# falcon-computing/falcon-genome

Measured on AMD Instinct MI355X. Metric: PairHMM GCUPS + banded-SW GCUPS per GPU; end-to-end htc regions/sec at 8 GPUs, higher is better.
Workload: dtype fp32 (fp64 rescue)

## Files before the change

falcon-genome_amd/csrc/fcship_api.cpp:

```cpp
#include <hip/hip_runtime.h>
#include <rocprim/device/device_radix_sort.hpp>

#include <algorithm>
#include <chrono>
#include <cmath>
#include <cstdlib>
#include <cstring>
#include <map>
#include <memory>
#include <condition_variable>
#include <mutex>
#include <thread>
#include <vector>

#include "fcship_internal.h"

namespace fcs {

static thread_local std::string g_last_error;
static thread_local int64_t g_last_rescued = 0;
static thread_local double g_last_device_ms = 0, g_last_rescue_ms = 0;
void set_error(const std::string& msg) { g_last_error = msg; }
int fail(int code, const std::string& msg) {
  set_error(msg);
// ... 469 lines not shown
  d.dq = b->read_dq;
  d.gq = b->read_gcp;
  d.read_off = b->read_off;
  d.read_len = b->read_len;
  d.hb = b->hap_bases;
  d.hap_off = b->hap_off;
  d.hap_len = b->hap_len;
  d.pair_read = b->pair_read;
  d.pair_hap = b->pair_hap;
  d.n_pairs = b->n_pairs;
  return d;
}

static int check_batch_shape(const fcs_phmm_batch* b) {
  if (!b) return fail(FCS_ERR_INVALID, "[E::fcship] null PairHMM batch");
  if (b->n_pairs < 0 || b->n_reads < 0 || b->n_haps < 0)
    return fail(FCS_ERR_INVALID, "[E::fcship] negative PairHMM batch size");
  if (b->n_pairs > 0x7FFFFFFF) return fail(FCS_ERR_UNSUPPORTED, "[E::fcship] more than 2^31-1 pairs per batch");
  if (b->n_pairs > 0 && (!b->read_bases || !b->read_bq || !b->read_iq || !b->read_dq || !b->read_gcp ||
                         !b->read_off || !b->read_len || !b->hap_bases || !b->hap_off || !b->hap_len ||
                         !b->pair_read || !b->pair_hap))
    return fail(FCS_ERR_INVALID, "[E::fcship] null pointer in PairHMM batch");
  if (b->max_hap_len < 0 || b->max_read_len < 0)
    return fail(FCS_ERR_INVALID, "[E::fcship] negative max length in PairHMM batch");
  return FCS_OK;
}

extern "C" {

const char* fcs_last_error(void) { return g_last_error.c_str(); }
const char* fcs_version(void) { return "fcship 0.1.0 (gfx950)"; }

int fcs_device_count(void) {
  int n = 0;
  if (hipGetDeviceCount(&n) != hipSuccess) return 0;
  return n;
}

int fcs_set_default_device(int32_t device) {
  int rc = check_device(device);
  if (rc) return rc;
  g_default_device = device;
  return FCS_OK;
}

void fcs_phmm_opts_default(fcs_phmm_opts* o) {
  if (!o) return;
  o->device = 0;
  o->use_fp64_rescue = 1;
  o->rescue_threshold = 1e-28f;
  o->exact_order = 0;
}

void fcs_bsw_params_default(fcs_bsw_params* p) {
  if (!p) return;
  for (int i = 0, k = 0; i < 4; ++i) {
    for (int j = 0; j < 4; ++j) p->mat[k++] = (int8_t)(i == j ? 1 : -4);
    p->mat[k++] = -1;
  }
  for (int j = 0; j < 5; ++j) p->mat[20 + j] = -1;
  p->o_del = 6;
  p->e_del = 1;
  p->o_ins = 6;
  p->e_ins = 1;
  p->end_bonus = 5;
  p->zdrop = 100;
}

int fcs_phmm_plan_create(int32_t device, int64_t max_pairs, fcs_phmm_plan** plan) {
  if (!plan || max_pairs < 0) return fail(FCS_ERR_INVALID, "[E::fcs_phmm_plan_create] bad arguments");
  int rc = check_device(device);
  if (rc) return rc;
  FCS_SET_DEVICE((device));
  DeviceTables* t = nullptr;
  rc = get_device_tables(device, &t);
  if (rc) return rc;
  std::unique_ptr<fcs_phmm_plan> p(new fcs_phmm_plan());
  p->device = device;
  p->max_pairs = max_pairs;
  const size_t n = (size_t)std::max<int64_t>(max_pairs, 1);
  FCS_HIP_CHECK(hipMalloc(&p->idx_out, n * 4));
  FCS_HIP_CHECK(hipMalloc(&p->rescue_list, n * 4));
  FCS_HIP_CHECK(hipMalloc(&p->fb_list, n * 4));
  FCS_HIP_CHECK(hipMalloc(&p->rescue_count, (2 + kPhmmLaunchClasses + 1) * sizeof(unsigned long long)));
  p->fb_count = p->rescue_count + 1;
  p->bounds = reinterpret_cast<int64_t*>(p->rescue_count + 2);
  constexpr size_t kBins = (size_t)1 << (kPhmmKeyBits - 4);
  FCS_HIP_CHECK(hipMalloc(&p->bin_hist, 2 * kBins * sizeof(uint32_t)));
  p->bin_cursor = p->bin_hist + kBins;
  *plan = p.release();
  return FCS_OK;
}

int fcs_phmm_plan_destroy(fcs_phmm_plan* p) {
  if (!p) return FCS_OK;
  ::fcs::DeviceScope dev_scope;
  (void)hipSetDevice(p->device);
  (void)hipFree(p->idx_out);
  (void)hipFree(p->rescue_list);
  (void)hipFree(p->fb_list);
  (void)hipFree(p->rescue_count);
  (void)hipFree(p->bin_hist);
  delete p;
  return FCS_OK;
}

int fcs_phmm_dev_schedule(fcs_phmm_plan* plan, const fcs_phmm_batch* b, void* stream) {
  if (!plan) return fail(FCS_ERR_INVALID, "[E::fcs_phmm_dev_schedule] null plan");
  int rc = check_batch_shape(b);
  if (rc) return rc;
  if (b->n_pairs > plan->max_pairs) return fail(FCS_ERR_INVALID, "[E::fcs_phmm_dev_schedule] batch exceeds plan");
  FCS_SET_DEVICE((plan->device));
  hipStream_t s = (hipStream_t)stream;
  const PhmmDevBatch d = to_dev(b);
  plan->scheduled = -1;
  if (!plan->bin_zeroed)
    FCS_HIP_CHECK(hipMemsetAsync(plan->bin_hist, 0, ((size_t)1 << (kPhmmKeyBits - 4)) * sizeof(uint32_t), s));
  plan->bin_zeroed = false;
  if ((rc = launch_phmm_bin_schedule(d, plan->idx_out, plan->bounds, plan->rescue_count, plan->bin_hist,
                                     plan->bin_cursor, s)))
    return rc;
  plan->bin_zeroed = true;
  plan->counters_zeroed = true;
  if (fault_drop_schedule()) FCS_HIP_CHECK(hipMemsetAsync(plan->bounds, 0, (kPhmmLaunchClasses + 1) * sizeof(int64_t), s));
  plan->scheduled = b->n_pairs;
  return FCS_OK;
}

int fcs_phmm_dev_forward(fcs_phmm_plan* plan, const fcs_phmm_batch* b, double* out, const fcs_phmm_opts* opts,
                         void* stream) {
  if (!plan || !opts) return fail(FCS_ERR_INVALID, "[E::fcs_phmm_dev_forward] null plan/opts");
  int rc = check_batch_shape(b);
  if (rc) return rc;
  if (plan->scheduled != b->n_pairs)
    return fail(FCS_ERR_INVALID, "[E::fcs_phmm_dev_forward] batch not scheduled (call fcs_phmm_dev_schedule)");
  if (b->n_pairs > 0 && !out) return fail(FCS_ERR_INVALID, "[E::fcs_phmm_dev_forward] null output");
  FCS_SET_DEVICE((plan->device));
  DeviceTables* t = nullptr;
  rc = get_device_tables(plan->device, &t);
  if (rc) return rc;
  hipStream_t s = (hipStream_t)stream;
  if (!plan->counters_zeroed)
    FCS_HIP_CHECK(hipMemsetAsync(plan->rescue_count, 0, 2 * sizeof(unsigned long long), s));
  plan->counters_zeroed = false;
  return launch_phmm_forward(to_dev(b), plan->idx_out, b->n_pairs, std::max(b->max_hap_len, 1), plan->bounds, *t,
                             opts->exact_order != 0, out, plan->rescue_list, plan->rescue_count,
                             opts->rescue_threshold, opts->use_fp64_rescue != 0, plan->fb_list, plan->fb_count, s);
}

int fcs_phmm_dev_rescue(fcs_phmm_plan* plan, const fcs_phmm_batch* b, double* out, const fcs_phmm_opts* opts,
                        void* stream) {
  if (!plan || !opts) return fail(FCS_ERR_INVALID, "[E::fcs_phmm_dev_rescue] null plan/opts");
  int rc = check_batch_shape(b);
  if (rc) return rc;
  if (!opts->use_fp64_rescue) return FCS_OK;
  FCS_SET_DEVICE((plan->device));
  DeviceTables* t = nullptr;
  rc = get_device_tables(plan->device, &t);
  if (rc) return rc;
  return launch_phmm_rescue(to_dev(b), plan->rescue_list, plan->rescue_count, b->n_pairs,
                            std::max(b->max_hap_len, 1), *t, opts->exact_order != 0, out, (hipStream_t)stream);
}

int fcs_phmm_dev_run(fcs_phmm_plan* plan, const fcs_phmm_batch* b, double* out, const fcs_phmm_opts* opts,
                     void* stream) {
  int rc = fcs_phmm_dev_schedule(plan, b, stream);
  if (rc) return rc;
  rc = fcs_phmm_dev_forward(plan, b, out, opts, stream);
  if (rc) return rc;
  return fcs_phmm_dev_rescue(plan, b, out, opts, stream);
}

int fcs_stream_release(int32_t device, void* stream) {
  int rc = check_device(device);
  if (rc) return rc;
  FCS_SET_DEVICE((device));
  ForkSet f;
  BswWorkspace ws;
  bool have_fork = false;
  {
    std::lock_guard<std::mutex> lk(g_fork_mu);
    auto wi = g_stream_ws->find({device, (hipStream_t)stream});
    if (wi != g_stream_ws->end()) {
      ws = wi->second;
      g_stream_ws->erase(wi);
    }
    auto it = g_fork_sets->find({device, (hipStream_t)stream});
    if (it != g_fork_sets->end()) {
      f = it->second;
      g_fork_sets->erase(it);
      have_fork = true;
    }
  }
  if (ws.keys_in) {
    (void)hipStreamSynchronize((hipStream_t)stream);
    ws_free(ws);
  }
  if (!have_fork) return FCS_OK;
  hipError_t first = hipSuccess;
  const char* what = nullptr;
  auto note = [&](hipError_t e, const char* w) {
    if (e != hipSuccess && first == hipSuccess) first = e, what = w;
  };
  for (int i = 0; i < kForkStreams - 1; ++i) {
    note(hipStreamSynchronize(f.side[i]), "hipStreamSynchronize");
    note(hipStreamDestroy(f.side[i]), "hipStreamDestroy");
    note(hipEventDestroy(f.join[i]), "hipEventDestroy");
  }
  note(hipEventDestroy(f.fork), "hipEventDestroy");
  if (first != hipSuccess)
    return fail(FCS_ERR_DEVICE, std::string("[E::fcs_stream_release] ") + what + ": " + hipGetErrorString(first));
  return FCS_OK;
}

int fcs_device_warmup(int32_t device, int32_t sessions) {
  int rc = check_device(device);
  if (rc) return rc;
  static const uint8_t b[1] = {'A'}, q[1] = {30}, g[1] = {10}, iq[1] = {45};
  const fcs_phmm_read r{b, q, iq, iq, g, 1};
  const fcs_phmm_hap h{b, 1};
  double out = 0;
  fcs_phmm_opts o;
  fcs_phmm_opts_default(&o);
  o.device = device;
  if ((rc = fcs_phmm_compute(&r, 1, &h, 1, &out, &o))) return rc;
  FCS_SET_DEVICE((device));
  return prefill_sessions(device, sessions <= 0 ? sessions_per_device() : sessions);
}

int fcs_phmm_last_device_ms(double* device_ms, double* rescue_ms) {
// ... 1066 lines not shown
```

falcon-genome_amd/csrc/fcship_internal.h:

```cpp
#pragma once

#include <hip/hip_runtime.h>
#include <stdint.h>

#include <string>

#include "fcship.h"

namespace fcs {

void set_error(const std::string& msg);
int fail(int code, const std::string& msg);
#define FCS_HIP_CHECK(expr)                                                                  \
  do {                                                                                       \
    hipError_t _e = (expr);                                                                  \
    if (_e != hipSuccess)                                                                    \
      return ::fcs::fail(FCS_ERR_DEVICE, std::string("[E::fcship] ") + #expr + ": " +        \
                                             hipGetErrorString(_e));                         \
  } while (0)

struct DeviceScope {
  int prev = -1;
  DeviceScope() {
    if (hipGetDevice(&prev) != hipSuccess) prev = -1;
// ... 33 lines not shown
  const long long o = __double_as_longlong(old), s = __double_as_longlong(src);
  const int lo = __builtin_amdgcn_update_dpp((int)o, (int)s, kDppRowShr1, 0xF, 0xF, false);
  const int hi = __builtin_amdgcn_update_dpp((int)(o >> 32), (int)(s >> 32), kDppRowShr1, 0xF, 0xF, false);
  return __longlong_as_double(((long long)hi << 32) | (unsigned int)lo);
}
template <typename T> __device__ __forceinline__ T dpp_row_shr1(T old, T src);
template <> __device__ __forceinline__ float dpp_row_shr1<float>(float old, float src) { return dpp_row_shr1_f(old, src); }
template <> __device__ __forceinline__ double dpp_row_shr1<double>(double old, double src) { return dpp_row_shr1_d(old, src); }

__device__ __forceinline__ int dpp_wave_shr1_i(int old, int src) {
  return __builtin_amdgcn_update_dpp(old, src, kDppWaveShr1, 0xF, 0xF, false);
}

__device__ __forceinline__ int wave_incl_max(int v, int neg) {
  v = max(v, __builtin_amdgcn_update_dpp(neg, v, kDppRowShr1, 0xF, 0xF, false));
  v = max(v, __builtin_amdgcn_update_dpp(neg, v, kDppRowShr2, 0xF, 0xF, false));
  v = max(v, __builtin_amdgcn_update_dpp(neg, v, kDppRowShr4, 0xF, 0xF, false));
  v = max(v, __builtin_amdgcn_update_dpp(neg, v, kDppRowShr8, 0xF, 0xF, false));
  v = max(v, __builtin_amdgcn_update_dpp(neg, v, kDppRowBcast15, 0xA, 0xF, false));
  v = max(v, __builtin_amdgcn_update_dpp(neg, v, kDppRowBcast31, 0xC, 0xF, false));
  return v;
}

__device__ __forceinline__ int lane_id() { return (int)__lane_id(); }

__device__ __forceinline__ int read_lane(int v, int lane) { return __builtin_amdgcn_readlane(v, lane); }
__device__ __forceinline__ int first_lane(int v) { return __builtin_amdgcn_readfirstlane(v); }

__device__ __forceinline__ int wave_max(int v) {
  return read_lane(wave_incl_max(v, INT32_MIN), 63);
}

__host__ __device__ __forceinline__ int bwa_max_gap(int qlen, int max_mat, int end_bonus, int o, int e) {
  if (e <= 0) return 0x7FFFFFFF;
  const int n = qlen * max_mat + end_bonus - o;
  const int m = (n + e) / e;
  return m > 1 ? m : 1;
}

template <typename T>
struct PhmmTables {
  const T* ph2pr;
  const T* dmatch;
  const T* dmis;
  const T* mm;
  T init_const;
  T log10_init;
};
constexpr int kMmEntries = (127 * 128) / 2 + 128;

struct PhmmDevBatch {
  const uint8_t *rb, *bq, *iq, *dq, *gq;
  const int64_t* read_off;
  const int32_t* read_len;
  const uint8_t* hb;
  const int64_t* hap_off;
  const int32_t* hap_len;
  const int32_t* pair_read;
  const int32_t* pair_hap;
  int64_t n_pairs;
};

struct DeviceTables {
  bool ready = false;
  float* f_tabs = nullptr;
  double* d_tabs = nullptr;
  PhmmTables<float> tf;
  PhmmTables<double> td;
};
int get_device_tables(int device, DeviceTables** out);

void build_phmm_tables_f(float* ph2pr, float* dmatch, float* dmis, float* mm);
void build_phmm_tables_d(double* ph2pr, double* dmatch, double* dmis, double* mm);

constexpr int kForkStreams = 4;
int fork_streams(hipStream_t s, hipStream_t (&fs)[kForkStreams]);
int join_streams(hipStream_t s, const hipStream_t (&fs)[kForkStreams]);

int launch_phmm_bin_schedule(const PhmmDevBatch& b, int32_t* idx_out, int64_t* bounds, unsigned long long* counters,
                             uint32_t* hist, uint32_t* cursor, hipStream_t s);
int launch_phmm_forward(const PhmmDevBatch& b, const int32_t* order, int64_t count, int max_hap_len,
                        const int64_t* bounds, const DeviceTables& t, bool exact, double* out, int32_t* rescue_list,
                        unsigned long long* rescue_count, float thr, bool use_rescue, int32_t* fb_list,
                        unsigned long long* fb_count, hipStream_t s);
int launch_phmm_rescue(const PhmmDevBatch& b, const int32_t* list, const unsigned long long* count_dev,
                       int64_t max_count, int max_hap_len, const DeviceTables& t, bool exact, double* out,
                       hipStream_t s);

struct BswDevBatch {
  const uint8_t* qbuf;
  const int64_t* qoff;
  const int32_t* qlen;
  const uint8_t* tbuf;
  const int64_t* toff;
  const int32_t* tlen;
  const int32_t* h0;
  const int32_t* w;
  int64_t n;
};
struct BswParams {
  int8_t mat[25];
  int32_t o_del, e_del, o_ins, e_ins, end_bonus, zdrop;
  int32_t max_mat;
  int32_t matpack[5];
  int32_t lane_ok;
  int32_t pair_ok;
  int32_t pair_bias;
  int32_t pair_cg;
  int32_t pair_k256, pair_one;
};
constexpr int kBswPairBucket0 = 10;
constexpr int kBswWideBucket = 15;
struct BswWorkspace {
  int64_t cap = 0;
  uint32_t* keys_in = nullptr;
  uint32_t* keys_out = nullptr;
  int32_t* idx_in = nullptr;
  int32_t* idx_out = nullptr;
  int64_t* bounds = nullptr;
  void* tmp = nullptr;
  size_t tmp_bytes = 0;
};
hipError_t sort_pairs_u32(void* tmp, size_t& bytes, const uint32_t* kin, uint32_t* kout, const int32_t* vin,
                          int32_t* vout, int n, hipStream_t s, int end_bit = 32);
constexpr int kBswKeyBucketShift = 20;
constexpr int kBswKeyBits = 24;
constexpr int kPhmmKeyClassShift = 12;
constexpr int kPhmmKeyBits = 16;
constexpr int kStreamClasses = 4;
constexpr int kPhmmClasses = 6;
constexpr int kLongClasses = 2;
constexpr int kColsLaunch = 8;
constexpr int kPhmmLaunchClasses = kLongClasses + kColsLaunch + kPhmmClasses;
int launch_bsw_extend_sorted(const BswDevBatch& b, const BswParams& p, int max_qlen, int max_tlen, int32_t* res,
                             int64_t* cells, const BswWorkspace& ws, hipStream_t s);
int launch_bsw_extend_wide(const BswDevBatch& b, const BswParams& p, int max_qlen, int max_tlen, int32_t* res,
                           int64_t* cells, const int32_t* order, const int64_t* bounds, hipStream_t s);
int launch_bsw_align(const BswDevBatch& b, const BswParams& p, const int32_t* xtra, int max_qlen, int max_tlen,
                     int32_t* out, hipStream_t s, bool all_u8);
int launch_bsw_global(const BswDevBatch& b, const BswParams& p, int max_qlen, int max_tlen, int32_t* scores,
                      uint8_t* zbuf, int64_t zbytes, const int64_t* zoff, uint32_t* cigar, const int64_t* cigar_off,
                      const int32_t* cigar_cap, int32_t* n_cigar, hipStream_t s);
int launch_bgzf_inflate(const uint8_t* comp, const int64_t* coff, const int64_t* uoff, int32_t n, uint8_t* out,
                        int32_t* status, hipStream_t s);

}
```

falcon-genome_amd/csrc/phmm_cols.h:

```cpp
#pragma once

namespace fcs {

constexpr int kColsClasses = 8;
constexpr int kColsMinR = 33;
__host__ __device__ constexpr int cols_C(int c) { return c == 0 ? 19 : 18 - c; }
__host__ __device__ constexpr int cols_hmax(int c) { return 16 * cols_C(c) - 1; }
__host__ __device__ inline int cols_class(int H) {
  for (int c = kColsClasses - 1; c >= 0; --c)
    if (H <= cols_hmax(c)) return c;
  return -1;
}
constexpr int kColsRing = 32;
constexpr int kColsChunks = 6;
constexpr int kColsChunkBytes = kColsRing * 4 * 16;
constexpr int kColsCapOff = kColsChunks * kColsChunkBytes;
constexpr int kColsTabOff = kColsCapOff + 4 * 8 * 8;
constexpr int kColsLds = kColsTabOff + 3 * 128 * 4;

__device__ __forceinline__ uint32_t vconst(uint32_t k) {
  uint32_t r;
  asm volatile("v_mov_b32 %0, %1" : "=v"(r) : "i"(k));
  return r;
}
// ... 657 lines not shown
          }
          asm volatile("" ::: "memory");
          const uint32_t a0 = xs + (uint32_t)(S * 8);
          const uint32_t pa = min(a0, a0 - (uint32_t)(kCols1Ring * 8)) + segoff;
          auto ld2 = [&](int chunk) {
            return *reinterpret_cast<const __attribute__((address_space(3))) pf2*>((uintptr_t)(pa + chunk * kCols1ChunkBytes));
          };
          const pf2 r0 = ld2(0), r1 = ld2(1), r2 = ld2(2), r3 = ld2(3);
          const pu2 cr = *reinterpret_cast<const __attribute__((address_space(3))) pu2*>((uintptr_t)(pa + 4 * kCols1ChunkBytes));
          const float e1 = r0.x, e3 = r0.y, my = r1.x, yy = r1.y, mm = r2.x, gm = r2.y, mx = r3.x, xx = r3.y;
          const float z = (float)(cr.y >> 24);
          const float din = __int_as_float(__builtin_amdgcn_update_dpp(__float_as_int(z), __float_as_int(dn), kDppRowShr1, 0xF, 0xF, false));
          const float xnx = __int_as_float(__builtin_amdgcn_update_dpp(__float_as_int(z), __float_as_int(xo), kDppRowShr1, 0xF, 0xF, false));
          const float xcur = xin;
          xin = xnx;
          uint32_t mA = 0;
          auto prior = [&](int j, const float dep) {
            if ((j & 3) == 0) mA = __builtin_amdgcn_perm(cr.y, cr.x, cur[j >> 2]);
            int a;
            asm volatile("v_bfe_i32 %0, %1, %2, 1" : "=v"(a) : "v"(mA), "i"(8 * (j & 3)), "v"(dep));
            return sel_v((uint32_t)a, e1, e3);
          };
          float Mn = xcur * prior(0, xcur);
          float D = din, Mp = 0.f, Dp = 0.f;
#pragma unroll
          for (int j = 0; j < C; ++j) {
            const float M = Mn;
            if (j > 0) D = __builtin_fmaf(Mp, my, Dp * yy);
            float I = In[j], Xo = Xn[j];
            asm volatile("" : "+v"(I), "+v"(Xo) : "v"(D));
            if (j + 1 < C) Mn = Xo * prior(j + 1, D);
            float xn = __builtin_fmaf(M, mm, __builtin_fmaf(I, gm, D));
            float in = __builtin_fmaf(M, mx, I * xx);
            asm volatile("" : "+v"(xn), "+v"(in));
            Xn[j] = xn;
            In[j] = in;
            Mp = M;
            Dp = D;
          }
          dn = __builtin_fmaf(Mp, my, Dp * yy);
          xo = Xn[C - 1];
          uint64_t keep;
          const uint32_t cpa = capa + 0u;
          const float dnv = dn;
          asm volatile(
              "s_mov_b64 %0, exec\n\t"
              "s_mov_b64 exec, %3\n\t"
              "ds_write_b32 %1, %2 offset:%4\n\t"
              "s_mov_b64 exec, %0"
              : "=&s"(keep)
              : "v"(cpa), "v"(dnv), "s"(kTopLanes), "i"(4 * S)
              : "memory");
        };
        [&]<int... S>(std::integer_sequence<int, S...>) {
          (step(std::integral_constant<int, S>{}), ...);
        }(std::make_integer_sequence<int, 8>{});
        g0 += 8;
        swmask >>= 8;
        capa += 32;
        xs += 64;
        xs = min(xs, xs - (uint32_t)(kCols1Ring * 8));
      }
      if (any_cap) {
        if (sl == 15 && (unsigned)(cap - gb) < 16u) {
          const float acc = *reinterpret_cast<const float*>(smem_raw + kCols1CapOff + seg * 64 + 4 * (cap - gb));
          const int p = capp;
          if (capo) {
            const unsigned long long k = atomicAdd(fb_count, 1ull);
            fb_list[k] = p;
            out[p] = __builtin_nan("");
          } else if (use_rescue && acc < thr) {
            const unsigned long long k = atomicAdd(rescue_count, 1ull);
            rescue_list[k] = p;
            out[p] = __builtin_nan("");
          } else {
            out[p] = (double)(log10f(acc) - tab.log10_init);
          }
        }
      }
    }
  }
}

}
```

falcon-genome_amd/csrc/phmm_kernels.hip:

```cpp
#include <hip/hip_runtime.h>

#include <algorithm>
#include <cstdlib>
#include <cstring>

#include <utility>

#include "fcship_internal.h"

namespace fcs {

constexpr int PFD = 2;
template <typename T> struct alignas(2 * sizeof(T)) PhRing {
  T X, I;
};

__device__ __forceinline__ float fma_t(float a, float b, float c) { return fmaf(a, b, c); }
__device__ __forceinline__ double fma_t(double a, double b, double c) { return fma(a, b, c); }

__device__ __forceinline__ unsigned char base_code(unsigned char b) {
  return b == 'A' ? 0 : b == 'C' ? 1 : b == 'G' ? 2 : b == 'T' ? 3 : b == 'N' ? 4 : 5;
}
__device__ __forceinline__ int base_mask(int rb) {
  const int c = base_code((unsigned char)rb);
// ... 287 lines not shown
        if (bytecmp)
          phmm_stripe<T, EXACT, true, true, W>(sp, ring, hapl, sl, (tend + 16) >> 4, lim, ulim, accM, accI, tab, nraw, nprm, top);
        else
          phmm_stripe<T, EXACT, true, false, W>(sp, ring, hapl, sl, (tend + 16) >> 4, lim, ulim, accM, accI, tab, nraw, nprm, top);
        if (seg_sums && sl == sum_lane) {
          const T sum = accM + accI;
          if constexpr (RESCUE_PASS) {
            out[p] = log10(sum) - (double)tab.log10_init;
          } else {
            if (use_rescue && sum < (T)thr) {
              const unsigned long long k = atomicAdd(rescue_count, 1ull);
              rescue_list[k] = p;
              out[p] = __builtin_nan("");
            } else {
              out[p] = (double)(log10f((float)sum) - (float)tab.log10_init);
            }
          }
        }
      } else {
        if (bytecmp)
          phmm_stripe<T, EXACT, false, true, W>(prm, ring, hapl, sl, (Hmax + W + 15) >> 4, -1, -1, accM, accI, tab, nraw, nprm, top);
        else
          phmm_stripe<T, EXACT, false, false, W>(prm, ring, hapl, sl, (Hmax + W + 15) >> 4, -1, -1, accM, accI, tab, nraw, nprm, top);
      }
      prm = nprm;
    }
  }
}

}

#include "phmm2.h"
#include "phmm_stream.h"
#include "phmm_cols.h"

namespace fcs {

static __host__ __device__ int nslot_for(int max_hap_len) { return ((max_hap_len + 51 + 15) / 16) * 16; }
static __host__ __device__ int nslot_for_w(int max_hap_len, int W) {
  return ((max_hap_len + 2 * W + 19 + 15) / 16) * 16;
}

static_assert(kPhmmLaunchClasses <= 16 && kPhmmKeyClassShift + 4 <= kPhmmKeyBits, "class fits the key");
__host__ __device__ inline int phmm_class(int H) {
  const int c = (nslot_for(H) - 224 + 31) / 32;
  return c < 0 ? 0 : c > kPhmmClasses - 1 ? kPhmmClasses - 1 : c;
}

__host__ __device__ inline int phmm_launch_class(int R, int H, int& stream_cls) {
  stream_cls = -1;
  if (R >= kStreamMinR && R <= kStreamMaxR && H >= 1) {
    static_assert(kColsMinR <= kStreamMinR, "column-blocked streams take every streamed read");
    const int cc = cols_class(H);
    stream_cls = cc >= 0 ? 0 : stream_class(H);
    if (cc >= 0) return kLongClasses + cc;
    if (stream_cls >= 2) return kStreamClasses - 1 - stream_cls;
    stream_cls = -1;
  }
  return kLongClasses + kColsLaunch + kPhmmClasses - 1 - phmm_class(max(H, 0));
}

__device__ __forceinline__ uint32_t phmm_key(const PhmmDevBatch& b, long long p) {
  const int R = b.read_len[b.pair_read[p]];
  const int H = b.hap_len[b.pair_hap[p]];
  int sc;
  const uint32_t cf = (uint32_t)phmm_launch_class(R, H, sc);
  const uint32_t hh = 0xFFFu - (uint32_t)min(max(H, 0), 0xFFF);
  uint32_t low;
  if (sc >= 0)
    low = hh;
  else
    low = ((3u - (uint32_t)min((max(R, 0) + 15) >> 4, 3)) << 10) | (0x3FFu - (uint32_t)min(max(H, 0) >> 2, 0x3FF));
  return (cf << kPhmmKeyClassShift) | low;
}

constexpr int kPhmmBins = 1 << (kPhmmKeyBits - 4);
constexpr int kBinBlock = 1024, kBinItems = 4;
__device__ __forceinline__ int phmm_bin(const PhmmDevBatch& b, long long p) { return (int)(phmm_key(b, p) >> 4); }

__global__ __launch_bounds__(kBinBlock) void phmm_bin_count_kernel(const PhmmDevBatch b, uint32_t* __restrict__ hist,
                                                                    unsigned long long* __restrict__ counters) {
  __shared__ uint32_t h[kPhmmBins];
  for (int i = threadIdx.x; i < kPhmmBins; i += kBinBlock) h[i] = 0;
  if (blockIdx.x == 0 && threadIdx.x == 0) {
    counters[0] = 0ull;
    counters[1] = 0ull;
  }
  __syncthreads();
  const long long base = (long long)blockIdx.x * (kBinBlock * kBinItems);
  for (int k = 0; k < kBinItems; ++k) {
    const long long p = base + (long long)k * kBinBlock + threadIdx.x;
    if (p < b.n_pairs) atomicAdd(&h[phmm_bin(b, p)], 1u);
  }
  __syncthreads();
  for (int i = threadIdx.x; i < kPhmmBins; i += kBinBlock)
    if (h[i]) atomicAdd(&hist[i], h[i]);
}

__global__ __launch_bounds__(kBinBlock) void phmm_bin_scan_kernel(uint32_t* __restrict__ hist,
                                                                   uint32_t* __restrict__ cursor, long long n,
                                                                   int64_t* __restrict__ bounds) {
  constexpr int kPer = kPhmmBins / kBinBlock;
  __shared__ uint32_t part[kBinBlock];
  const int t = threadIdx.x;
  uint32_t v[kPer], sum = 0;
  for (int j = 0; j < kPer; ++j) {
    v[j] = hist[t * kPer + j];
    sum += v[j];
  }
  part[t] = sum;
  __syncthreads();
  for (int off = 1; off < kBinBlock; off <<= 1) {
    const uint32_t x = t >= off ? part[t - off] : 0u;
    __syncthreads();
    part[t] += x;
    __syncthreads();
  }
  uint32_t run = part[t] - sum;
  for (int j = 0; j < kPer; ++j) {
    const int bin = t * kPer + j;
    cursor[bin] = run;
    if ((bin & 255) == 0 && (bin >> 8) < kPhmmLaunchClasses) bounds[bin >> 8] = run;
    run += v[j];
    hist[bin] = 0u;
  }
  if (t == 0) bounds[kPhmmLaunchClasses] = n;
}

__global__ __launch_bounds__(kBinBlock) void phmm_bin_scatter_kernel(const PhmmDevBatch b,
                                                                      uint32_t* __restrict__ cursor,
                                                                      int32_t* __restrict__ idx) {
  __shared__ uint32_t cnt[kPhmmBins], at[kPhmmBins];
  for (int i = threadIdx.x; i < kPhmmBins; i += kBinBlock) cnt[i] = 0;
  __syncthreads();
  const long long base = (long long)blockIdx.x * (kBinBlock * kBinItems);
  int bin[kBinItems];
  uint32_t rank[kBinItems];
  for (int k = 0; k < kBinItems; ++k) {
    const long long p = base + (long long)k * kBinBlock + threadIdx.x;
    bin[k] = p < b.n_pairs ? phmm_bin(b, p) : -1;
    rank[k] = bin[k] >= 0 ? atomicAdd(&cnt[bin[k]], 1u) : 0u;
  }
  __syncthreads();
  for (int i = threadIdx.x; i < kPhmmBins; i += kBinBlock)
    if (cnt[i]) at[i] = atomicAdd(&cursor[i], cnt[i]);
  __syncthreads();
  for (int k = 0; k < kBinItems; ++k)
    if (bin[k] >= 0) idx[at[bin[k]] + rank[k]] = (int32_t)(base + (long long)k * kBinBlock + threadIdx.x);
}

int launch_phmm_bin_schedule(const PhmmDevBatch& b, int32_t* idx_out, int64_t* bounds, unsigned long long* counters,
                             uint32_t* hist, uint32_t* cursor, hipStream_t s) {
  static_assert(kPhmmBins % kBinBlock == 0 && (kPhmmLaunchClasses << 8) <= kPhmmBins, "bins");
  const long long n = b.n_pairs > 0 ? b.n_pairs : 0;
  const unsigned nb = (unsigned)std::max<long long>((n + kBinBlock * kBinItems - 1) / (kBinBlock * kBinItems), 1);
  hipLaunchKernelGGL(phmm_bin_count_kernel, dim3(nb), dim3(kBinBlock), 0, s, b, hist, counters);
  FCS_HIP_CHECK(hipGetLastError());
  hipLaunchKernelGGL(phmm_bin_scan_kernel, dim3(1), dim3(kBinBlock), 0, s, hist, cursor, n, bounds);
  FCS_HIP_CHECK(hipGetLastError());
  if (n > 0) {
    hipLaunchKernelGGL(phmm_bin_scatter_kernel, dim3(nb), dim3(kBinBlock), 0, s, b, cursor, idx_out);
    FCS_HIP_CHECK(hipGetLastError());
  }
  return FCS_OK;
}

constexpr size_t kLdsBytes = 160 * 1024;

template <typename T, bool EXACT, bool RESCUE, int W = 16>
static int launch_one(const PhmmDevBatch& b, const int32_t* order, const unsigned long long* count_dev,
                      long long count_host, const int64_t* bounds, int cls, int nslot, long long max_groups,
                      const PhmmTables<T>& tab, double* out, int32_t* rescue_list, unsigned long long* rescue_count,
                      float thr, bool use_rescue, hipStream_t s) {
  int nseg = 64 / W;
  size_t lds = (size_t)nseg * (ring_stride<T>(nslot) + nslot);
  if (lds > kLdsBytes && nseg > 1) {
    nseg = 1;
    lds = (size_t)ring_stride<T>(nslot) + nslot;
    max_groups *= 4;
  }
  if (lds > kLdsBytes)
    return fail(FCS_ERR_UNSUPPORTED, "[E::fcship] haplotype too long for the LDS boundary ring (max_hap_len " +
                                         std::to_string(nslot - 67) + ")");
  auto kern = phmm_kernel<T, EXACT, RESCUE, W>;
  if (lds > 64 * 1024)
    FCS_HIP_CHECK(hipFuncSetAttribute((const void*)kern, hipFuncAttributeMaxDynamicSharedMemorySize, (int)lds));
  long long grid = max_groups;
  const long long cap = 65536;
  if (grid > cap) grid = cap;
  if (grid < 1) grid = 1;
  hipLaunchKernelGGL(kern, dim3((unsigned)grid), dim3(64), lds, s, b, order, count_dev, count_host, bounds, cls, nslot,
                     tab, out, rescue_list, rescue_count, thr, use_rescue ? 1 : 0, nseg);
  FCS_HIP_CHECK(hipGetLastError());
  return FCS_OK;
}

static int stream_pairs_per_segment(int64_t n) {
  static const int forced = [] {
    const char* e = std::getenv("FCSHIP_STREAM_K");
    return e ? std::atoi(e) : 0;
  }();
  if (forced > 0) return std::min(forced, kStreamMaxK);
  const int64_t k = n / (4 * 24576);
  return (int)std::max<int64_t>(1, std::min<int64_t>(kStreamMaxK, k));
}

static int cols_pairs_per_half(int64_t n) {
  static const int forced = [] {
    const char* e = std::getenv("FCSHIP_STREAM_K");
    return e ? std::atoi(e) : 0;
  }();
  if (forced > 0) return std::min(forced, 8);
  const int64_t k = n / (8 * 24576);
  return (int)std::max<int64_t>(1, std::min<int64_t>(8, k));
}

static int cols1_forced_k() {
  static const int forced = [] {
    const char* e = std::getenv("FCSHIP_STREAM_K");
    return e ? std::atoi(e) : 0;
  }();
  return forced > 0 ? std::min(forced, kCols1MaxK) : 0;
}
static int cols1_pairs_per_stream(int64_t n) {
  if (const int f = cols1_forced_k()) return f;
  const int64_t k = n / (4 * 32768);
  return (int)std::max<int64_t>(1, std::min<int64_t>(kCols1MaxK, k));
}

static bool cols_single(int c) {
  static const int forced = [] {
    const char* e = std::getenv("FCSHIP_COLS");
    if (!e) return 0;
    return !std::strcmp(e, "single") ? 1 : !std::strcmp(e, "packed") ? 2 : 0;
  }();
  if (forced) return forced == 1;
  static constexpr bool kSingle[kColsClasses] = {true, true, true, true, true, true, true, true};
  return kSingle[c];
}

int launch_phmm_forward(const PhmmDevBatch& b, const int32_t* order, int64_t count, int max_hap_len,
                        const int64_t* bounds, const DeviceTables& t, bool exact, double* out, int32_t* rescue_list,
                        unsigned long long* rescue_count, float thr, bool use_rescue, int32_t* fb_list,
                        unsigned long long* fb_count, hipStream_t s) {
  if (count <= 0) return FCS_OK;
  const long long groups = (count + 3) / 4;
  const int ns_max = nslot_for(max_hap_len);
  const int c_max = phmm_class(max_hap_len);
  hipStream_t fs[kForkStreams];
  if (const int rc = fork_streams(s, fs); rc != FCS_OK) return rc;
  int fork = 0;
  for (int j = 0; j < kLongClasses; ++j) {
    const int sc = kStreamClasses - 1 - j;
    const int lo = j == 0 ? stream_class_hmax(sc - 1) : cols_hmax(0);
    if (max_hap_len <= lo) continue;
    const int hmax = std::min(stream_class_hmax(sc), max_hap_len);
    hipStream_t st = fs[fork++ % kForkStreams];
    if (exact) {
      const int rc = launch_one<float, true, false>(b, order, nullptr, count, bounds, j, nslot_for(hmax), groups, t.tf,
                                                   out, rescue_list, rescue_count, thr, use_rescue, st);
      if (rc != FCS_OK) return rc;
      continue;
    }
    const size_t lds = (size_t)stream_lds(hmax);
    if (lds > kLdsBytes) return fail(FCS_ERR_UNSUPPORTED, "[E::fcship] streamed PairHMM class exceeds LDS");
    const int K = stream_pairs_per_segment(count);
    const int w = stream_class_waves(sc);
    const int tail = 2 * 4 * 1024 * w;
    const unsigned grid = (unsigned)std::min<long long>(
        std::max<long long>((count + 4 * K - 1) / (4 * K) + (tail + 3) / 4, 1), 65536);
    auto launch = [&](auto kern) -> int {
      if (lds > 64 * 1024)
        FCS_HIP_CHECK(hipFuncSetAttribute((const void*)kern, hipFuncAttributeMaxDynamicSharedMemorySize, (int)lds));
      hipLaunchKernelGGL(kern, dim3(grid), dim3(64), lds, st, b, order, bounds, j, K, tail, stream_nslot(hmax),
                         stream_hstride(hmax), t.tf, out, rescue_list, rescue_count, thr, use_rescue ? 1 : 0, fb_list,
                         fb_count);
      FCS_HIP_CHECK(hipGetLastError());
      return FCS_OK;
    };
    const int rc = w >= 3 ? launch(phmm3_kernel<3>) : w == 2 ? launch(phmm3_kernel<2>) : launch(phmm3_kernel<1>);
    if (rc != FCS_OK) return rc;
  }
  for (int c = 0; c < kColsLaunch; ++c) {
    const int lo = c + 1 < kColsLaunch ? cols_hmax(c + 1) : 0;
    if (max_hap_len <= lo) continue;
    const int j = kLongClasses + c;
    hipStream_t st = fs[fork++ % kForkStreams];
    if (exact) {
      const int rc = launch_one<float, true, false>(b, order, nullptr, count, bounds, j,
                                                   nslot_for(std::min(cols_hmax(c), max_hap_len)), groups, t.tf, out,
                                                   rescue_list, rescue_count, thr, use_rescue, st);
      if (rc != FCS_OK) return rc;
      continue;
    }
    if (cols_single(c)) {
      const int K = cols1_pairs_per_stream(count);
      const int tail = cols1_forced_k() ? 4 : 1024 * cols1_waves(cols_C(c)) * 4;
      const unsigned grid = (unsigned)std::min<long long>(
          std::max<long long>((count + 4 * K - 1) / (4 * K) + (tail + 3) / 4, 1), 65536);
      auto launch = [&](auto kern) -> int {
        hipLaunchKernelGGL(kern, dim3(grid), dim3(64), (size_t)kCols1Lds, st, b, order, bounds, j, K, tail, t.tf, out,
                           rescue_list, rescue_count, thr, use_rescue ? 1 : 0, fb_list, fb_count);
        FCS_HIP_CHECK(hipGetLastError());
        return FCS_OK;
      };
      static_assert(cols_C(0) == 19 && cols_C(1) == 17 && cols_C(7) == 11 && kColsClasses == 8, "launch table below");
      int rc;
      switch (cols_C(c)) {
        case 19: rc = launch(phmm5_kernel<19>); break;
        case 17: rc = launch(phmm5_kernel<17>); break;
        case 16: rc = launch(phmm5_kernel<16>); break;
        case 15: rc = launch(phmm5_kernel<15>); break;
        case 14: rc = launch(phmm5_kernel<14>); break;
        case 13: rc = launch(phmm5_kernel<13>); break;
        case 12: rc = launch(phmm5_kernel<12>); break;
        default: rc = launch(phmm5_kernel<11>); break;
      }
      if (rc != FCS_OK) return rc;
      continue;
    }
    const int K = cols_pairs_per_half(count);
    const int tail = 1024 * 3 * 8;
    const unsigned grid = (unsigned)std::min<long long>(
        std::max<long long>((count + 8 * K - 1) / (8 * K) + (tail + 7) / 8, 1), 65536);
    auto launch = [&](auto kern) -> int {
      hipLaunchKernelGGL(kern, dim3(grid), dim3(64), (size_t)kColsLds, st, b, order, bounds, j, K, tail, t.tf, out,
                         rescue_list, rescue_count, thr, use_rescue ? 1 : 0, fb_list, fb_count);
      FCS_HIP_CHECK(hipGetLastError());
      return FCS_OK;
    };
    static_assert(cols_C(0) == 19 && cols_C(1) == 17 && cols_C(7) == 11 && kColsClasses == 8, "launch table below");
    int rc;
    switch (cols_C(c)) {
      case 19: rc = launch(phmm4_kernel<19>); break;
      case 17: rc = launch(phmm4_kernel<17>); break;
      case 16: rc = launch(phmm4_kernel<16>); break;
      case 15: rc = launch(phmm4_kernel<15>); break;
      case 14: rc = launch(phmm4_kernel<14>); break;
      case 13: rc = launch(phmm4_kernel<13>); break;
      case 12: rc = launch(phmm4_kernel<12>); break;
      default: rc = launch(phmm4_kernel<11>); break;
    }
    if (rc != FCS_OK) return rc;
  }
  constexpr long long kGroupedGrid = 8192;
  int gfork = 0;
  for (int j = kPhmmClasses - 1 - c_max; j < kPhmmClasses; ++j) {
    const int c = kPhmmClasses - 1 - j;
    const int lc = kLongClasses + kColsLaunch + j;
    const int ns = (c == kPhmmClasses - 1) ? ns_max : std::min(224 + 32 * c, ns_max);
    hipStream_t st = fs[1 + gfork++ % (kForkStreams - 1)];
    const int ns2 = ns + 16;
    const size_t lds2 = (size_t)phmm2_lds(ns2);
    if (!exact && lds2 <= kLdsBytes) {
      if (lds2 > 64 * 1024)
        FCS_HIP_CHECK(
            hipFuncSetAttribute((const void*)phmm2_kernel, hipFuncAttributeMaxDynamicSharedMemorySize, (int)lds2));
      const unsigned grid = (unsigned)std::min<long long>(std::max<long long>(groups, 1), kGroupedGrid);
      hipLaunchKernelGGL(phmm2_kernel, dim3(grid), dim3(64), lds2, st, b, order, bounds, lc, ns2, t.tf, out,
                         rescue_list, rescue_count, thr, use_rescue ? 1 : 0);
      FCS_HIP_CHECK(hipGetLastError());
      continue;
    }
    const int rc = exact ? launch_one<float, true, false>(b, order, nullptr, count, bounds, lc, ns, groups, t.tf, out,
                                                           rescue_list, rescue_count, thr, use_rescue, st)
                         : launch_one<float, false, false>(b, order, nullptr, count, bounds, lc, ns, groups, t.tf, out,
                                                            rescue_list, rescue_count, thr, use_rescue, st);
    if (rc != FCS_OK) return rc;
  }
  if (const int rc = join_streams(s, fs); rc != FCS_OK) return rc;
  if (exact) return FCS_OK;
  return launch_one<float, false, false>(b, fb_list, fb_count, 0, nullptr, 0, ns_max,
                                         std::min<long long>(groups, 2048), t.tf, out, rescue_list, rescue_count, thr,
                                         use_rescue, s);
}

int launch_phmm_rescue(const PhmmDevBatch& b, const int32_t* list, const unsigned long long* count_dev,
                       int64_t max_count, int max_hap_len, const DeviceTables& t, bool exact, double* out,
// ... 22 lines not shown
```

Baseline: 4535.

## Add persistent work-queue PairHMM column kernel with atomic per-class queue heads

Adds a persistent phmm6 kernel for the column classes. A fixed grid of waves, sized to the CU count, pulls pairs dynamically from a per-class atomic queue head instead of using a static per-wave partition with a tail scheme. New pairs are fetched ahead of need so a segment can stream one pair after another with little idle time. The counter buffer grows to hold the queue heads, which are zeroed alongside the existing counters. The aim is better load balance across uneven pair lengths, paid for with atomic contention and more complex control flow.

```diff
diff --git a/falcon-genome_amd/csrc/fcship_api.cpp b/falcon-genome_amd/csrc/fcship_api.cpp
--- a/falcon-genome_amd/csrc/fcship_api.cpp
+++ b/falcon-genome_amd/csrc/fcship_api.cpp
@@ -575,9 +575,9 @@
   FCS_HIP_CHECK(hipMalloc(&p->idx_out, n * 4));
   FCS_HIP_CHECK(hipMalloc(&p->rescue_list, n * 4));
   FCS_HIP_CHECK(hipMalloc(&p->fb_list, n * 4));
-  FCS_HIP_CHECK(hipMalloc(&p->rescue_count, (2 + kPhmmLaunchClasses + 1) * sizeof(unsigned long long)));
+  FCS_HIP_CHECK(hipMalloc(&p->rescue_count, (kPhmmCounters + kPhmmLaunchClasses + 1) * sizeof(unsigned long long)));
   p->fb_count = p->rescue_count + 1;
-  p->bounds = reinterpret_cast<int64_t*>(p->rescue_count + 2);
+  p->bounds = reinterpret_cast<int64_t*>(p->rescue_count + kPhmmCounters);
   constexpr size_t kBins = (size_t)1 << (kPhmmKeyBits - 4);
   FCS_HIP_CHECK(hipMalloc(&p->bin_hist, 2 * kBins * sizeof(uint32_t)));
   p->bin_cursor = p->bin_hist + kBins;
@@ -634,11 +634,12 @@
   if (rc) return rc;
   hipStream_t s = (hipStream_t)stream;
   if (!plan->counters_zeroed)
-    FCS_HIP_CHECK(hipMemsetAsync(plan->rescue_count, 0, 2 * sizeof(unsigned long long), s));
+    FCS_HIP_CHECK(hipMemsetAsync(plan->rescue_count, 0, kPhmmCounters * sizeof(unsigned long long), s));
   plan->counters_zeroed = false;
   return launch_phmm_forward(to_dev(b), plan->idx_out, b->n_pairs, std::max(b->max_hap_len, 1), plan->bounds, *t,
                              opts->exact_order != 0, out, plan->rescue_list, plan->rescue_count,
-                             opts->rescue_threshold, opts->use_fp64_rescue != 0, plan->fb_list, plan->fb_count, s);
+                             opts->rescue_threshold, opts->use_fp64_rescue != 0, plan->fb_list, plan->fb_count,
+                             plan->rescue_count + kPhmmQueueHead0, s);
 }
 
 int fcs_phmm_dev_rescue(fcs_phmm_plan* plan, const fcs_phmm_batch* b, double* out, const fcs_phmm_opts* opts,
diff --git a/falcon-genome_amd/csrc/fcship_internal.h b/falcon-genome_amd/csrc/fcship_internal.h
--- a/falcon-genome_amd/csrc/fcship_internal.h
+++ b/falcon-genome_amd/csrc/fcship_internal.h
@@ -139,7 +139,7 @@
 int launch_phmm_forward(const PhmmDevBatch& b, const int32_t* order, int64_t count, int max_hap_len,
                         const int64_t* bounds, const DeviceTables& t, bool exact, double* out, int32_t* rescue_list,
                         unsigned long long* rescue_count, float thr, bool use_rescue, int32_t* fb_list,
-                        unsigned long long* fb_count, hipStream_t s);
+                        unsigned long long* fb_count, unsigned long long* qheads, hipStream_t s);
 int launch_phmm_rescue(const PhmmDevBatch& b, const int32_t* list, const unsigned long long* count_dev,
                        int64_t max_count, int max_hap_len, const DeviceTables& t, bool exact, double* out,
                        hipStream_t s);
@@ -189,6 +189,8 @@
 constexpr int kLongClasses = 2;
 constexpr int kColsLaunch = 8;
 constexpr int kPhmmLaunchClasses = kLongClasses + kColsLaunch + kPhmmClasses;
+constexpr int kPhmmQueueHead0 = 2;
+constexpr int kPhmmCounters = kPhmmQueueHead0 + kColsLaunch;
 int launch_bsw_extend_sorted(const BswDevBatch& b, const BswParams& p, int max_qlen, int max_tlen, int32_t* res,
                              int64_t* cells, const BswWorkspace& ws, hipStream_t s);
 int launch_bsw_extend_wide(const BswDevBatch& b, const BswParams& p, int max_qlen, int max_tlen, int32_t* res,
diff --git a/falcon-genome_amd/csrc/phmm_cols.h b/falcon-genome_amd/csrc/phmm_cols.h
--- a/falcon-genome_amd/csrc/phmm_cols.h
+++ b/falcon-genome_amd/csrc/phmm_cols.h
@@ -763,4 +763,321 @@
   }
 }
 
+constexpr int kCols6Lds = kCols1Lds;
+constexpr int kCols6Waves = 3;
+constexpr int kCols6Ahead = 48;
+static_assert(kCols6Lds <= 13653, "12 waves per CU");
+
+template <int C>
+__global__ __launch_bounds__(64, kCols6Waves) void phmm6_kernel(
+    const PhmmDevBatch b, const int32_t* __restrict__ order, const int64_t* __restrict__ bounds, const int cls,
+    const PhmmTables<float> gtab, double* __restrict__ out, int32_t* __restrict__ rescue_list,
+    unsigned long long* __restrict__ rescue_count, const float thr, const int use_rescue,
+    int32_t* __restrict__ fb_list, unsigned long long* __restrict__ fb_count,
+    unsigned long long* __restrict__ qhead) {
+  constexpr int NW = (C + 3) / 4;
+  constexpr int kNever = 0x3FFFFFFF;
+  extern __shared__ __align__(16) unsigned char smem_raw[];
+  const int lane = threadIdx.x;
+  const int seg = lane >> 4;
+  const int sl = lane & 15;
+  const int sbase = lane & 48;
+  const int i0 = sl * C;
+  const int64_t cbeg = bounds[cls];
+  const long long count = bounds[cls + 1] - cbeg;
+  order += cbeg;
+  unsigned pend = 0xFu;
+  uint32_t qv = 0u;
+  if (lane == 0) qv = (uint32_t)atomicAdd(qhead, 4ull);
+  if ((long long)(uint32_t)__builtin_amdgcn_readfirstlane((int)qv) >= count) return;
+  PhmmTables<float> tab = gtab;
+  {
+    float* const t = reinterpret_cast<float*>(smem_raw + kCols1TabOff);
+    for (int i = lane; i < 128; i += 64) {
+      t[i] = gtab.ph2pr[i];
+      t[128 + i] = gtab.dmatch[i];
+      t[256 + i] = gtab.dmis[i];
+    }
+    tab.ph2pr = t;
+    tab.dmatch = t + 128;
+    tab.dmis = t + 256;
+  }
+
+  int pm = -1, Rm = 0, Hm = 0, Gm = 0;
+  int64_t rom = 0, hom = 0;
+  float Im = 0.f;
+  int nq = 0, gend = 0;
+  bool closed = false;
+  unsigned other = 0u;
+  int sb = sbase * 4;
+  auto bp = [&](int v, int k) { return __builtin_amdgcn_ds_bpermute(sb + 4 * (k & 15), v); };
+  auto tG = [&](int k) { return bp(Gm, k); };
+  auto tR = [&](int k) { return bp(Rm, k); };
+  auto tH = [&](int k) { return bp(Hm, k); };
+  auto tP = [&](int k) { return bp(pm, k); };
+  auto tI = [&](int k) { return __int_as_float(bp(__float_as_int(Im), k)); };
+  auto t64 = [&](int64_t v, int k) {
+    const int lo = bp((int)v, k), hi = bp((int)(v >> 32), k);
+    return (int64_t)(((uint64_t)(uint32_t)hi << 32) | (uint32_t)lo);
+  };
+  auto valid = [&](int k) { return k >= 0 && k < nq; };
+  auto complete = [&](int gmin) {
+    const long long base = (long long)(uint32_t)__builtin_amdgcn_readfirstlane((int)qv);
+    const bool mine = (pend >> seg) & 1u;
+    const long long idx = base + __popc(pend & ((1u << seg) - 1u));
+    const bool got = mine && idx < count;
+    if (mine && !got) closed = true;
+    if (got) {
+      const int p = order[idx];
+      const int ri = b.pair_read[p], hi = b.pair_hap[p];
+      const int R = b.read_len[ri], H = b.hap_len[hi];
+      const int G = max(gend, gmin);
+      if (sl == (nq & 15)) {
+        pm = p;
+        Rm = R;
+        Hm = H;
+        rom = b.read_off[ri];
+        hom = b.hap_off[hi];
+        Im = tab.init_const / (float)H;
+        Gm = G;
+      }
+      other &= ~(1u << (nq & 15));
+      gend = G + R + 2;
+      ++nq;
+    }
+    pend = 0u;
+  };
+
+  uint32_t cur[NW], nxt[NW];
+  int nk = -1, swr = kNever;
+  auto fetch_codes = [&](int k, uint32_t (&dst)[NW]) {
+    const bool ok = valid(k);
+    const int Hk = tH(k);
+    const int H = ok ? Hk : 0;
+    const int64_t ho = t64(hom, k);
+    uint32_t raw[NW + 1];
+    int al;
+    cols_load<NW>(b.hb, ok ? ho : 0, H, i0, raw, al);
+    bool oth = false;
+    cols_convert<NW>(raw, al, i0, H, dst, oth);
+    const unsigned long long bal = __ballot(oth && ok);
+    if (((bal >> sbase) & 0xFFFFull) != 0ull) other |= 1u << (k & 15);
+  };
+#pragma unroll
+  for (int d = 0; d < NW; ++d) cur[d] = nxt[d] = 0x06060606u;
+  int kc = 0, cap, capp;
+  auto load_cap = [&] {
+    const bool ok = valid(kc);
+    const int v = tG(kc) + tR(kc);
+    cap = ok ? v : -kNever;
+    capp = tP(kc);
+  };
+
+  int kp = 0;
+  RawRow praw{-1, 0, 0, 0, 0, 0, 0};
+  int prole = 0;
+  float pih = 0.f;
+  bool kok = false, nok = false;
+  int kG = 0, kR = 0, nG = 0;
+  float kI = 0.f;
+  int64_t kro = 0;
+  auto load_cursor = [&] {
+    kok = valid(kp);
+    kG = tG(kp);
+    kR = tR(kp);
+    kI = tI(kp);
+    kro = t64(rom, kp);
+    nok = valid(kp + 1);
+    nG = tG(kp + 1);
+  };
+  auto stage_a = [&](int base) {
+    const int g = base + sl;
+    const bool adv = nok && g >= nG;
+    if (__ballot(adv) != 0ull) {
+      if (adv) ++kp;
+      load_cursor();
+    }
+    const int r = g - kG;
+    int role = 0;
+    if (kok && r >= 0 && r < kR) role = r == kR - 1 ? 3 : 2;
+    else if (kok && r == kR) role = 4;
+    pih = kI;
+    prole = role | (r == 0 ? 16 : 0);
+    praw = (role == 2 || role == 3) ? load_raw(b, kR, kro, r) : RawRow{-1, 0, 0, 0, 0, 0, 0};
+  };
+  auto stage_b = [&](int base) {
+    cols1_put(smem_raw, (int)((unsigned)(base + sl) % (unsigned)kCols1Ring), seg,
+              cols_item(tab, praw, prole & 15, (prole & 16) != 0, pih));
+  };
+  {
+    complete(0);
+    load_cursor();
+    load_cap();
+    cols1_put(smem_raw, 32 + sl, seg, cols_item(tab, RawRow{-1, 0, 0, 0, 0, 0, 0}, 0, false, 0.f));
+    stage_a(0);
+    stage_b(0);
+    stage_a(16);
+  }
+
+  float Xn[C], In[C];
+#pragma unroll
+  for (int j = 0; j < C; ++j) {
+    Xn[j] = 1.f;
+    In[j] = 0.f;
+  }
+  float dn = 1.f, xo = 1.f, xin = 1.f;
+  const uint32_t segoff = (uint32_t)seg * (kCols1Ring * 8u) + lds_addr(smem_raw);
+
+  for (int t0 = 0;; t0 += 16) {
+    asm volatile("" : "+v"(sb));
+    if (pend != 0u) {
+      complete(t0 + 32);
+      load_cursor();
+      load_cap();
+    }
+    {
+      const bool need = !closed && gend < t0 + 32 + kCols6Ahead && nq - kc < 8;
+      const unsigned long long bal = __ballot(need && sl == 0);
+      if (bal != 0ull) {
+        pend = (unsigned)((bal & 1ull) | ((bal >> 15) & 2ull) | ((bal >> 30) & 4ull) | ((bal >> 45) & 8ull));
+        qv = 0u;
+        if (lane == 0) qv = (uint32_t)atomicAdd(qhead, (unsigned long long)__popc(pend));
+      }
+    }
+    {
+      if (swr != kNever && swr + 16 <= t0) swr = kNever;
+      const bool ev = swr == kNever && nk + 1 < nq;
+      if (__ballot(ev) != 0ull) {
+        uint32_t tmp[NW];
+        fetch_codes(nk + 1, tmp);
+        const int gn = tG(nk + 1);
+        if (ev) {
+#pragma unroll
+          for (int d = 0; d < NW; ++d) nxt[d] = tmp[d];
+          ++nk;
+          swr = gn;
+        }
+      }
+    }
+    stage_b(t0 + 16);
+    stage_a(t0 + 32);
+    {
+      const bool adv = cap >= 0 && cap + 15 < t0;
+      if (__ballot(adv) != 0ull) {
+        if (adv) ++kc;
+        load_cap();
+      }
+    }
+    if (__ballot(!closed || kc < nq) == 0ull) break;
+    const bool capo = (other >> (kc & 15)) & 1u;
+    const int gb = t0 - sl;
+    const bool any_cap = __ballot(sl == 15 && (unsigned)(cap - gb) < 16u) != 0ull;
+    unsigned swmask = 0u;
+#pragma unroll
+    for (int q = 0; q < 4; ++q) {
+      const int lo = __builtin_amdgcn_readlane(swr, 16 * q) - t0;
+      if (lo < 16 && lo + 15 >= 0) {
+        const int a = max(lo, 0), bnd = min(lo + 15, 15);
+        swmask |= ((2u << bnd) - 1u) & ~((1u << a) - 1u);
+      }
+    }
+    uint32_t xs = ((uint32_t)(gb + kCols1Ring) % (uint32_t)kCols1Ring) * 8u;
+    uint32_t capa = lds_addr(smem_raw) + kCols1CapOff + seg * 64;
+    int g0 = gb;
+
+#pragma nounroll
+    for (int pass = 0; pass < 2; ++pass) {
+      auto step = [&](auto S_) {
+        constexpr int S = decltype(S_)::value;
+        const int g = g0 + S;
+        if (swmask & (1u << S)) {
+          const bool take = g == swr;
+#pragma unroll
+          for (int d = 0; d < NW; ++d) {
+            uint32_t r;
+            asm("v_cndmask_b32_e64 %0, %1, %2, %3" : "=v"(r) : "v"(cur[d]), "v"(nxt[d]), "s"(__ballot(take)));
+            cur[d] = r;
+          }
+        }
+        asm volatile("" ::: "memory");
+        const uint32_t a0 = xs + (uint32_t)(S * 8);
+        const uint32_t pa = min(a0, a0 - (uint32_t)(kCols1Ring * 8)) + segoff;
+        auto ld2 = [&](int chunk) {
+          return *reinterpret_cast<const __attribute__((address_space(3))) pf2*>((uintptr_t)(pa + chunk * kCols1ChunkBytes));
+        };
+        const pf2 r0 = ld2(0), r1 = ld2(1), r2 = ld2(2), r3 = ld2(3);
+        const pu2 cr = *reinterpret_cast<const __attribute__((address_space(3))) pu2*>((uintptr_t)(pa + 4 * kCols1ChunkBytes));
+        const float e1 = r0.x, e3 = r0.y, my = r1.x, yy = r1.y, mm = r2.x, gm = r2.y, mx = r3.x, xx = r3.y;
+        const float z = (float)(cr.y >> 24);
+        const float din = __int_as_float(__builtin_amdgcn_update_dpp(__float_as_int(z), __float_as_int(dn), kDppRowShr1, 0xF, 0xF, false));
+        const float xnx = __int_as_float(__builtin_amdgcn_update_dpp(__float_as_int(z), __float_as_int(xo), kDppRowShr1, 0xF, 0xF, false));
+        const float xcur = xin;
+        xin = xnx;
+        uint32_t mA = 0;
+        auto prior = [&](int j, const float dep) {
+          if ((j & 3) == 0) mA = __builtin_amdgcn_perm(cr.y, cr.x, cur[j >> 2]);
+          int a;
+          asm volatile("v_bfe_i32 %0, %1, %2, 1" : "=v"(a) : "v"(mA), "i"(8 * (j & 3)), "v"(dep));
+          return sel_v((uint32_t)a, e1, e3);
+        };
+        float Mn = xcur * prior(0, xcur);
+        float D = din, Mp = 0.f, Dp = 0.f;
+#pragma unroll
+        for (int j = 0; j < C; ++j) {
+          const float M = Mn;
+          if (j > 0) D = __builtin_fmaf(Mp, my, Dp * yy);
+          float I = In[j], Xo = Xn[j];
+          asm volatile("" : "+v"(I), "+v"(Xo) : "v"(D));
+          if (j + 1 < C) Mn = Xo * prior(j + 1, D);
+          float xn = __builtin_fmaf(M, mm, __builtin_fmaf(I, gm, D));
+          float in = __builtin_fmaf(M, mx, I * xx);
+          asm volatile("" : "+v"(xn), "+v"(in));
+          Xn[j] = xn;
+          In[j] = in;
+          Mp = M;
+          Dp = D;
+        }
+        dn = __builtin_fmaf(Mp, my, Dp * yy);
+        xo = Xn[C - 1];
+        uint64_t keep;
+        const uint32_t cpa = capa + 0u;
+        const float dnv = dn;
+        asm volatile(
+            "s_mov_b64 %0, exec\n\t"
+            "s_mov_b64 exec, %3\n\t"
+            "ds_write_b32 %1, %2 offset:%4\n\t"
+            "s_mov_b64 exec, %0"
+            : "=&s"(keep)
+            : "v"(cpa), "v"(dnv), "s"(kTopLanes), "i"(4 * S)
+            : "memory");
+      };
+      [&]<int... S>(std::integer_sequence<int, S...>) {
+        (step(std::integral_constant<int, S>{}), ...);
+      }(std::make_integer_sequence<int, 8>{});
+      g0 += 8;
+      swmask >>= 8;
+      capa += 32;
+      xs += 64;
+      xs = min(xs, xs - (uint32_t)(kCols1Ring * 8));
+    }
+    if (any_cap) {
+      if (sl == 15 && (unsigned)(cap - gb) < 16u) {
+        const float acc = *reinterpret_cast<const float*>(smem_raw + kCols1CapOff + seg * 64 + 4 * (cap - gb));
+        const int p = capp;
+        if (capo) {
+          const unsigned long long k = atomicAdd(fb_count, 1ull);
+          fb_list[k] = p;
+          out[p] = __builtin_nan("");
+        } else if (use_rescue && acc < thr) {
+          const unsigned long long k = atomicAdd(rescue_count, 1ull);
+          rescue_list[k] = p;
+          out[p] = __builtin_nan("");
+        } else {
+          out[p] = (double)(log10f(acc) - tab.log10_init);
+        }
+      }
+    }
+  }
 }
+
+}
diff --git a/falcon-genome_amd/csrc/phmm_kernels.hip b/falcon-genome_amd/csrc/phmm_kernels.hip
--- a/falcon-genome_amd/csrc/phmm_kernels.hip
+++ b/falcon-genome_amd/csrc/phmm_kernels.hip
@@ -393,10 +393,7 @@
                                                                     unsigned long long* __restrict__ counters) {
   __shared__ uint32_t h[kPhmmBins];
   for (int i = threadIdx.x; i < kPhmmBins; i += kBinBlock) h[i] = 0;
-  if (blockIdx.x == 0 && threadIdx.x == 0) {
-    counters[0] = 0ull;
-    counters[1] = 0ull;
-  }
+  if (blockIdx.x == 0 && threadIdx.x < kPhmmCounters) counters[threadIdx.x] = 0ull;
   __syncthreads();
   const long long base = (long long)blockIdx.x * (kBinBlock * kBinItems);
   for (int k = 0; k < kBinItems; ++k) {
@@ -539,21 +536,42 @@
   return (int)std::max<int64_t>(1, std::min<int64_t>(kCols1MaxK, k));
 }
 
-static bool cols_single(int c) {
+enum ColsKernel { kColsPacked = 0, kColsSingle = 1, kColsQueue = 2 };
+static ColsKernel cols_kernel(int c) {
   static const int forced = [] {
     const char* e = std::getenv("FCSHIP_COLS");
-    if (!e) return 0;
-    return !std::strcmp(e, "single") ? 1 : !std::strcmp(e, "packed") ? 2 : 0;
+    if (!e) return -1;
+    return !std::strcmp(e, "queue")    ? (int)kColsQueue
+           : !std::strcmp(e, "single") ? (int)kColsSingle
+           : !std::strcmp(e, "packed") ? (int)kColsPacked
+                                       : -1;
   }();
-  if (forced) return forced == 1;
-  static constexpr bool kSingle[kColsClasses] = {true, true, true, true, true, true, true, true};
-  return kSingle[c];
+  if (forced >= 0) return (ColsKernel)forced;
+  static constexpr ColsKernel kDefault[kColsClasses] = {kColsQueue, kColsQueue, kColsQueue, kColsQueue,
+                                                        kColsQueue, kColsQueue, kColsQueue, kColsQueue};
+  return kDefault[c];
+}
+
+static int cols6_forced_waves() {
+  static const int forced = [] {
+    const char* e = std::getenv("FCSHIP_QUEUE_WAVES");
+    return e ? std::atoi(e) : 0;
+  }();
+  return forced > 0 ? forced : 0;
+}
+static int cols6_grid() {
+  if (const int f = cols6_forced_waves()) return f;
+  int dev = 0, cus = 0;
+  if (hipGetDevice(&dev) != hipSuccess ||
+      hipDeviceGetAttribute(&cus, hipDeviceAttributeMultiprocessorCount, dev) != hipSuccess || cus <= 0)
+    cus = 256;
+  return cus * 4 * kCols6Waves;
 }
 
 int launch_phmm_forward(const PhmmDevBatch& b, const int32_t* order, int64_t count, int max_hap_len,
                         const int64_t* bounds, const DeviceTables& t, bool exact, double* out, int32_t* rescue_list,
                         unsigned long long* rescue_count, float thr, bool use_rescue, int32_t* fb_list,
-                        unsigned long long* fb_count, hipStream_t s) {
+                        unsigned long long* fb_count, unsigned long long* qheads, hipStream_t s) {
   if (count <= 0) return FCS_OK;
   const long long groups = (count + 3) / 4;
   const int ns_max = nslot_for(max_hap_len);
@@ -604,7 +622,33 @@
       if (rc != FCS_OK) return rc;
       continue;
     }
-    if (cols_single(c)) {
+    const ColsKernel ck = cols_kernel(c);
+    if (ck == kColsQueue) {
+      const unsigned grid = (unsigned)cols6_grid();
+      auto launch = [&](auto kern) -> int {
+        hipLaunchKernelGGL(kern, dim3(grid), dim3(64), (size_t)kCols6Lds, st, b, order, bounds, j, t.tf, out,
+                           rescue_list, rescue_count, thr, use_rescue ? 1 : 0, fb_list, fb_count, qheads + c);
+        FCS_HIP_CHECK(hipGetLastError());
+        return FCS_OK;
+      };
+      static_assert(cols_C(0) == 19 && cols_C(1) == 17 && cols_C(7) == 11 && kColsClasses == 8 &&
+                        kColsLaunch == kColsClasses,
+                    "launch table below, one head word per class");
+      int rc;
+      switch (cols_C(c)) {
+        case 19: rc = launch(phmm6_kernel<19>); break;
+        case 17: rc = launch(phmm6_kernel<17>); break;
+        case 16: rc = launch(phmm6_kernel<16>); break;
+        case 15: rc = launch(phmm6_kernel<15>); break;
+        case 14: rc = launch(phmm6_kernel<14>); break;
+        case 13: rc = launch(phmm6_kernel<13>); break;
+        case 12: rc = launch(phmm6_kernel<12>); break;
+        default: rc = launch(phmm6_kernel<11>); break;
+      }
+      if (rc != FCS_OK) return rc;
+      continue;
+    }
+    if (ck == kColsSingle) {
       const int K = cols1_pairs_per_stream(count);
       const int tail = cols1_forced_k() ? 4 : 1024 * cols1_waves(cols_C(c)) * 4;
       const unsigned grid = (unsigned)std::min<long long>(
```

Result: faster. 4631 (median of 6 runs) (+2.1%).
